# HKUST-Aerial-Robotics/VINS-Mobile

Hardware: AMD Instinct MI355X
Metric: VIO frames/sec (KLT+window solve), 640x480/150 feats/W=10 (higher is better)
Workload: dtype f64 (solve) / u8+i32+f32 (KLT)

## Files before the change

### vins-mobile_amd/csrc/marg_core.h

```cpp
#pragma once

#include "solver_core.h"

namespace vio {

struct MargOut {
  int *n;
  int *kind, *index, *offset;
  double *x0;
  double *J;
  double *r;
  double *scratch;
  int ncap;
};

template <class MP>
struct MargWorkT {
  MP Am;
  int ld;
  ldsd bm;
  ldsd tol;
  ldsd ldinv;
  ldsd hff, gf, einv;
  ldsd prdx, prr;
// ... 329 lines not shown
    }
    const int mdrop = pos;
    auto keep = [&](int kind, int idx, int col, int new_index) {
      out.kind[nblocks] = kind, out.index[nblocks] = new_index, out.offset[nblocks] = col - mdrop;
      double *x0 = out.x0 + 9 * nblocks;
      for (int q = 0; q < 9; q++) x0[q] = 0.0;
      cldsd src = kind == 0 ? xpose + 7 * idx : kind == 1 ? xsb + 9 * idx : ex;
      int gs = kind == 1 ? 9 : 7;
      for (int q = 0; q < gs; q++) x0[q] = src[q];
      nblocks++;
    };
    for (int i = 0; i < P; i++)
      if (m.col_pose[i] == -2) {
        m.col_pose[i] = pos;
        keep(0, i, pos, flag == 0 ? i - 1 : (i == W ? W - 1 : i));
        pos += 6;
      }
    for (int i = 0; i < P; i++)
      if (m.col_sb[i] == -2) {
        m.col_sb[i] = pos;
        keep(1, i, pos, flag == 0 ? i - 1 : (i == W ? W - 1 : i));
        pos += 9;
      }
    if (m.col_ex[0] == -2) {
      m.col_ex[0] = pos;
      keep(2, 0, pos, 0);
      pos += 6;
    }
    m.meta[0] = pos, m.meta[1] = mdrop, m.meta[2] = pos - mdrop, m.meta[3] = nblocks;
  }
  VIO_SYNC();
  const int pos = m.meta[0], mdrop = m.meta[1], n = m.meta[2], nblocks = m.meta[3];
  const int ld = m.ld;
  if (pos > ld || n > out.ncap) {
    if (cx.tid == 0) out.n[0] = -2, out.n[1] = 0, out.n[2] = mdrop, out.n[3] = pos;
    return;
  }
  VIO_PARFOR(q, (int)tri_doubles(pos)) m.Am[q] = 0.0;
  VIO_PARFOR(q, pos) m.bm[q] = 0.0;
  VIO_PARFOR(f, F) m.hff[f] = 0.0, m.gf[f] = 0.0;
  if (flag == 0) VIO_PARFOR(q, 12 * F) {
    const int f = q / 12, c = q - 12 * f;
    v.WTf[(size_t)f * v.n6cap + (c < 6 ? c : 6 * P + c - 6)] = 0.0;
  }
  VIO_SYNC();
  if (pn > 0) {
    VIO_PARFOR(b, v.prior_nb) {
      int kind = v.pr_kind[b], idx = v.pr_index[b], o = v.pr_offset[b];
      const double *x0 = v.pr_x0 + 9 * b;
      int base = kind == 0 ? m.col_pose[idx] : kind == 1 ? m.col_sb[idx] : m.col_ex[0];
      int ls = kind == 1 ? 9 : 6;
      for (int k = 0; k < ls; k++) m.pcol[o + k] = base + k;
      if (kind == 0) prior_block_dx(7, xpose + 7 * idx, x0, m.prdx + o);
      else if (kind == 1) prior_block_dx(9, xsb + 9 * idx, x0, m.prdx + o);
      else prior_block_dx(7, ex, x0, m.prdx + o);
    }
    VIO_PARFOR(i, pn) m.prr[i] = v.prb0[i];
    VIO_SYNC();
    dense_matvec_cols(cx, v.prH0, pn, m.prdx, [&](int i, double sacc) { VIO_ATOMIC_ADD(m.prr + i, sacc); });
    {
      constexpr int kU = 12;
      const int nst = (pn + kU - 1) / kU;
      VIO_PARFOR(q, pn * nst) {
        const int a = q / nst, b0 = kU * (q - a * nst);
        const int ca = m.pcol[a];
        double x[kU];
#pragma unroll
        for (int u = 0; u < kU; u++) x[u] = v.prH0[a * pn + (b0 + u < pn ? b0 + u : b0)];
        VIO_SCHED_FENCE();
#pragma unroll
        for (int u = 0; u < kU; u++) {
          if (b0 + u >= pn) continue;
          const int cb = m.pcol[b0 + u];
          if (ca >= cb) m.Am[tri_at(ca, cb)] = x[u];
        }
      }
    }
    VIO_SYNC();
    VIO_PARFOR(a, pn) m.bm[m.pcol[a]] += m.prr[a];
    VIO_SYNC();
  }
  stamp(cx, ST_M_PRIOR);
  if (flag == 0) {
    if (cx.tid == 0)
      imu_eval_raw(v.gravity, v.preint, xpose, xsb, xpose + 7, xsb + 9, v.imu_r, v.imu_J);
    VIO_SYNC();
    VIO_PARFOR(r, 15) {
      const double *info = v.imu_info + r * 15;
      double s = 0;
      for (int k = 0; k < 15; k++) s += info[k] * v.imu_r[k];
      v.imu_Mr[r] = s;
    }
    VIO_PARFOR(q, 450) {
      int r = q / 30, c = q % 30;
      const double *info = v.imu_info + r * 15;
      double s = 0;
      for (int k = 0; k < 15; k++) s += info[k] * v.imu_J[k * 30 + c];
      v.imu_M[q] = s;
    }
    VIO_SYNC();
    VIO_PARFOR(q, 900) {
      int a = q / 30, b = q % 30;
      int ca = a < 6 ? m.col_pose[0] + a : a < 15 ? m.col_sb[0] + a - 6 : a < 21 ? m.col_pose[1] + a - 15 : m.col_sb[1] + a - 21;
      int cb = b < 6 ? m.col_pose[0] + b : b < 15 ? m.col_sb[0] + b - 6 : b < 21 ? m.col_pose[1] + b - 15 : m.col_sb[1] + b - 21;
      double s = 0;
      for (int k = 0; k < 15; k++) s += v.imu_J[k * 30 + a] * v.imu_M[k * 30 + b];
      if (ca >= cb) VIO_ATOMIC_ADD(m.Am + tri_at(ca, cb), s);
    }
    VIO_PARFOR(a, 30) {
      int ca = a < 6 ? m.col_pose[0] + a : a < 15 ? m.col_sb[0] + a - 6 : a < 21 ? m.col_pose[1] + a - 15 : m.col_sb[1] + a - 21;
      double s = 0;
      for (int k = 0; k < 15; k++) s += v.imu_J[k * 30 + a] * v.imu_Mr[k];
      VIO_ATOMIC_ADD(m.bm + ca, s);
    }
    stamp(cx, ST_M_IMU);
    const double cc = 1.0 / v.cauchy_b;
    int S0 = 0, nb0 = 0;
    for (int p = 0; p < v.npairs && v.pair_h[p] == 0; p++)
      if (v.pair_t[p] != P) S0 = (v.pair_s1[p] + 1) & ~1, nb0 = p + 1;
    auto G = m.stage;
    const int CH = m.stage_slots;
    if (CH < 2) {
      if (cx.tid == 0) out.n[0] = -3, out.n[1] = 0;
      return;
    }
    auto add_lower = [&](int ra, int ca, double val) {
      if (ra >= ca) VIO_ATOMIC_ADD(m.Am + tri_at(ra, ca), val);
      else VIO_ATOMIC_ADD(m.Am + tri_at(ca, ra), val);
    };
    const int lane_d = VIO_TID(cx) & 63;
    const bool dv = lane_d < nb0;
    const int d_s0 = dv ? v.pair_s0[lane_d] : 0, d_s1 = dv ? v.pair_s1[lane_d] : 0;
    const int d_t = dv ? ((v.pair_h[lane_d] != 0 || v.pair_t[lane_d] == P) ? -1 : v.pair_t[lane_d]) : -1;
    for (int c0 = 0; c0 < S0; c0 += CH) {
      VIO_PARFOR(slot, (S0 - c0 < CH ? S0 - c0 : CH)) {
        const int rec = v.srec_i[c0 + slot];
        double pij[6];
#pragma unroll
        for (int c = 0; c < 6; c++) pij[c] = v.srec_d[6 * (size_t)(c0 + slot) + c];
        if (rec < 0) continue;
        const int t = (rec >> 8) & 255, f = rec >> 16;
        if ((rec & 255) != 0 || t == P) continue;
        double r[2], Ji[12], Jj[12], Jex[12], Jl[2];
        projection_eval(v.s_info, xpose, xpose + 7 * t, ex, xfeat[f], pij, pij + 3, true, r, Ji, Jj, Jex, Jl);
        double sq = r[0] * r[0] + r[1] * r[1];
        double sr = sqrt(1.0 / (1.0 + sq * cc));
        auto g = G + slot * kMargSlot; auto gx = g + kSlotStride;
#pragma unroll
        for (int rr = 0; rr < 2; rr++) {
#pragma unroll
          for (int c = 0; c < 6; c++) {
            g[rr * kRowLen + c] = Ji[rr * 6 + c] * sr, g[rr * kRowLen + 6 + c] = Jj[rr * 6 + c] * sr;
            gx[rr * kMargRowX + c] = Jex[rr * 6 + c] * sr;
          }
          g[rr * kRowLen + 12] = r[rr] * sr, g[rr * kRowLen + 13] = Jl[rr] * sr;
        }
        const double s2 = sr * sr;
        double *wf = v.WTf + (size_t)f * v.n6cap;
#pragma unroll
        for (int c = 0; c < 6; c++) {
          wf[6 * t + c] = (Jj[c] * Jl[0] + Jj[6 + c] * Jl[1]) * s2;
          VIO_ATOMIC_ADD(wf + c, (Ji[c] * Jl[0] + Ji[6 + c] * Jl[1]) * s2);
          VIO_ATOMIC_ADD(wf + 6 * P + c, (Jex[c] * Jl[0] + Jex[6 + c] * Jl[1]) * s2);
        }
        VIO_ATOMIC_ADD(m.hff + f, (Jl[0] * Jl[0] + Jl[1] * Jl[1]) * s2);
        VIO_ATOMIC_ADD(m.gf + f, (Jl[0] * r[0] + Jl[1] * r[1]) * s2);
      }
      VIO_SYNC();
// ... 127 lines not shown
```

### vins-mobile_amd/csrc/solver_core.h

```cpp
#pragma once

#include <math.h>
#include <stdint.h>

#include <type_traits>

#include "vio_math.h"

#if defined(VIO_EMUL) || defined(VIO_SIMT)
#define VIO_HOST_BUILD 1
#endif
#ifdef VIO_HOST_BUILD
#define VIO_DEV inline
#define VIO_ATOMIC_ADD(p, v) ::vio::atomic_add((p), (v))
#else
#define VIO_DEV __device__ __forceinline__
#define VIO_ATOMIC_ADD(p, v) ::vio::atomic_add((p), (v))
#endif
#if defined(VIO_EMUL)
#define VIO_SYNC() ((void)0)
#define VIO_SYNC_LDS() ((void)0)
#elif defined(VIO_SIMT)
#define VIO_SYNC() __syncthreads()
#define VIO_SYNC_LDS() __syncthreads()
// ... 552 lines not shown
  const double sum_dt = pre[0];
  const double *delta_p = pre + 1, *delta_q = pre + 4, *delta_v = pre + 8, *lin_ba = pre + 11, *lin_bg = pre + 14;
  const double *J = pre + 17;
  PA Pi = pose_i, Pj = pose_j, Vi = sb_i, Bai = sb_i + 3, Bgi = sb_i + 6, Vj = sb_j, Baj = sb_j + 3, Bgj = sb_j + 6;
  Quat Qi{pose_i[3], pose_i[4], pose_i[5], pose_i[6]}, Qj{pose_j[3], pose_j[4], pose_j[5], pose_j[6]};
  Quat dq{delta_q[0], delta_q[1], delta_q[2], delta_q[3]};
  double dp_dba[9], dp_dbg[9], dq_dbg[9], dv_dba[9], dv_dbg[9];
  for (int i = 0; i < 3; i++)
    for (int j = 0; j < 3; j++) {
      dp_dba[i * 3 + j] = J[(0 + i) * 15 + 9 + j];
      dp_dbg[i * 3 + j] = J[(0 + i) * 15 + 12 + j];
      dq_dbg[i * 3 + j] = J[(3 + i) * 15 + 12 + j];
      dv_dba[i * 3 + j] = J[(6 + i) * 15 + 9 + j];
      dv_dbg[i * 3 + j] = J[(6 + i) * 15 + 12 + j];
    }
  double dba[3], dbg[3], th[3], t1[3], t2[3], cdv[3], cdp[3];
  for (int k = 0; k < 3; k++) dba[k] = Bai[k] - lin_ba[k], dbg[k] = Bgi[k] - lin_bg[k];
  mat3vec(dq_dbg, dbg, th);
  Quat cdq = qmul(dq, Quat{th[0] / 2.0, th[1] / 2.0, th[2] / 2.0, 1.0});
  mat3vec(dv_dba, dba, t1), mat3vec(dv_dbg, dbg, t2);
  for (int k = 0; k < 3; k++) cdv[k] = delta_v[k] + t1[k] + t2[k];
  mat3vec(dp_dba, dba, t1), mat3vec(dp_dbg, dbg, t2);
  for (int k = 0; k < 3; k++) cdp[k] = delta_p[k] + t1[k] + t2[k];
  const double T = sum_dt;
  const double G[3] = {0, 0, gravity};
  Quat Qi_inv = qinv(Qi);
  double a[3], b[3], ra[3], rb[3];
  for (int k = 0; k < 3; k++) {
    a[k] = 0.5 * G[k] * T * T + Pj[k] - Pi[k] - Vi[k] * T;
    b[k] = G[k] * T + Vj[k] - Vi[k];
  }
  qrot(Qi_inv, a, ra), qrot(Qi_inv, b, rb);
  Quat qr = qmul(qinv(cdq), qmul(Qi_inv, Qj));
  for (int k = 0; k < 3; k++) {
    res[0 + k] = ra[k] - cdp[k];
    res[6 + k] = rb[k] - cdv[k];
    res[9 + k] = Baj[k] - Bai[k];
    res[12 + k] = Bgj[k] - Bgi[k];
  }
  res[3] = 2 * qr.x, res[4] = 2 * qr.y, res[5] = 2 * qr.z;
  if (!Jraw) return;
  double Rinv[9], M[9], S[9], Mq[9];
  qtoR(Qi_inv, Rinv);
  const int ld = 30, cpi = 0, csi = 6, cpj = 15, csj = 21;
  for (int i = 0; i < 3; i++)
    for (int j = 0; j < 3; j++) Jraw[(0 + i) * ld + cpi + j] = -Rinv[i * 3 + j];
  skew3(ra, S);
  for (int i = 0; i < 3; i++)
    for (int j = 0; j < 3; j++) Jraw[(0 + i) * ld + cpi + 3 + j] = S[i * 3 + j];
  qleft_qright33(qmul(qinv(Qj), Qi), cdq, M);
  for (int i = 0; i < 3; i++)
    for (int j = 0; j < 3; j++) Jraw[(3 + i) * ld + cpi + 3 + j] = -M[i * 3 + j];
  skew3(rb, S);
  for (int i = 0; i < 3; i++)
    for (int j = 0; j < 3; j++) Jraw[(6 + i) * ld + cpi + 3 + j] = S[i * 3 + j];
  for (int i = 0; i < 3; i++)
    for (int j = 0; j < 3; j++) {
      Jraw[(0 + i) * ld + csi + 0 + j] = -Rinv[i * 3 + j] * T;
      Jraw[(0 + i) * ld + csi + 3 + j] = -dp_dba[i * 3 + j];
      Jraw[(0 + i) * ld + csi + 6 + j] = -dp_dbg[i * 3 + j];
      Jraw[(6 + i) * ld + csi + 0 + j] = -Rinv[i * 3 + j];
      Jraw[(6 + i) * ld + csi + 3 + j] = -dv_dba[i * 3 + j];
      Jraw[(6 + i) * ld + csi + 6 + j] = -dv_dbg[i * 3 + j];
      Jraw[(9 + i) * ld + csi + 3 + j] = -(double)(i == j);
      Jraw[(12 + i) * ld + csi + 6 + j] = -(double)(i == j);
    }
  qleft33(qmul(qmul(qinv(Qj), Qi), cdq), M);
  mat3mul(M, dq_dbg, Mq);
  for (int i = 0; i < 3; i++)
    for (int j = 0; j < 3; j++) Jraw[(3 + i) * ld + csi + 6 + j] = -Mq[i * 3 + j];
  for (int i = 0; i < 3; i++)
    for (int j = 0; j < 3; j++) Jraw[(0 + i) * ld + cpj + j] = Rinv[i * 3 + j];
  qleft33(qmul(qmul(qinv(cdq), Qi_inv), Qj), M);
  for (int i = 0; i < 3; i++)
    for (int j = 0; j < 3; j++) Jraw[(3 + i) * ld + cpj + 3 + j] = M[i * 3 + j];
  for (int i = 0; i < 3; i++)
    for (int j = 0; j < 3; j++) {
      Jraw[(6 + i) * ld + csj + 0 + j] = Rinv[i * 3 + j];
      Jraw[(9 + i) * ld + csj + 3 + j] = (double)(i == j);
      Jraw[(12 + i) * ld + csj + 6 + j] = (double)(i == j);
    }
}

template <class PX, class PD>
VIO_DEV void prior_block_dx(int gsize, PX x, const double *x0, PD dx) {
  if (gsize != 7) {
    for (int k = 0; k < gsize; k++) dx[k] = x[k] - x0[k];
    return;
  }
  for (int k = 0; k < 3; k++) dx[k] = x[k] - x0[k];
  Quat q = qmul(qinv(qfrom_pose(x0)), Quat{x[3], x[4], x[5], x[6]});
  double sgn = (q.w >= 0) ? 1.0 : -1.0;
  dx[3] = sgn * 2.0 * q.x, dx[4] = sgn * 2.0 * q.y, dx[5] = sgn * 2.0 * q.z;
}


#ifdef VIO_EMUL
template <class MP>
VIO_DEV void setup_imu_info(const Ctx &cx, const WinView &v, MP) {
  const int W = v.W;
  VIO_PARFOR(q, W * 450) {
    int f = q / 450, e = q % 450, r = e / 30, c = e % 30;
    v.imu_aug[q] = c < 15 ? v.preint[f * kPreintDoubles + 242 + r * 15 + c] : (double)(c - 15 == r);
  }
  VIO_SYNC();
  for (int c = 0; c < 15; c++) {
    VIO_PARFOR(f, W) {
      double *A = v.imu_aug + f * 450;
      int piv = c;
      for (int r = c + 1; r < 15; r++)
        if (fabs(A[r * 30 + c]) > fabs(A[piv * 30 + c])) piv = r;
      if (piv != c)
        for (int j = 0; j < 30; j++) {
          double t = A[c * 30 + j];
          A[c * 30 + j] = A[piv * 30 + j];
          A[piv * 30 + j] = t;
        }
      double d = A[c * 30 + c];
      for (int j = 0; j < 30; j++) A[c * 30 + j] /= d;
      for (int r = 0; r < 15; r++) v.imu_Mr[f * 15 + r] = A[r * 30 + c];
    }
    VIO_SYNC();
    VIO_PARFOR(q, W * 450) {
      int f = q / 450, e = q % 450, r = e / 30, j = e % 30;
      if (r != c) {
        double fac = v.imu_Mr[f * 15 + r];
        if (fac != 0.0) v.imu_aug[q] -= fac * v.imu_aug[f * 450 + c * 30 + j];
      }
    }
    VIO_SYNC();
  }
  VIO_PARFOR(q, W * 225) {
    int f = q / 225, e = q % 225, r = e / 15, c = e % 15;
    int rr = r >= c ? r : c, cc = r >= c ? c : r;
    v.imu_info[q] = v.imu_aug[f * 450 + rr * 30 + 15 + cc];
  }
  VIO_PARFOR(q, W * 450) v.imu_J[q] = 0.0;
  VIO_SYNC();
}
#else
template <class MP>
VIO_DEV void setup_imu_info_gj(const Ctx &cx, const WinView &v, MP mbox) {
  const int W = v.W;
  const int tid_ = VIO_TID(cx), j = tid_ & 31, slot = tid_ >> 5, nslots = cx.nt >> 5;
  for (int f0 = 0; f0 < W; f0 += nslots) {
    const int f = f0 + slot;
    const bool act = f < W && j < 30;
    const int fc = f < W ? f : 0;
    auto mb = mbox + slot * 32;
    double x[15];
#pragma unroll
    for (int r = 0; r < 15; r++)
      x[r] = j < 15 ? v.preint[fc * kPreintDoubles + 242 + r * 15 + (j < 15 ? j : 0)] : (double)(j - 15 == r);
#pragma unroll
    for (int c = 0; c < 15; c++) {
      if (j == c) {
        int piv = c;
        double best = fabs(x[c]);
#pragma unroll
        for (int r = c + 1; r < 15; r++)
          if (fabs(x[r]) > best) best = fabs(x[r]), piv = r;
#pragma unroll
        for (int r = 0; r < 15; r++) mb[r] = x[r];
        mb[15] = (double)piv;
      }
      __builtin_amdgcn_fence(__ATOMIC_RELEASE, "wavefront");
// ... 393 lines not shown
    const bool ok = m < nvalid && n < nvalid;
    const int hi = m > n ? m : n, lo = m > n ? n : m;
    A[r] = D[ok ? hi * ld + lo : 0];
  }
  tile_load_op_raw(Lprev, ld, nvalid, n, kq, l);
  VIO_SCHED_FENCE();
#pragma unroll
  for (int r = 0; r < 4; r++) {
    const int m = kq + 4 * r;
    A[r] = (m < nvalid && n < nvalid) ? A[r] : 0.0;
    E[r] = (m == n) ? 1.0 : 0.0;
  }
  if (with_update) {
    tile_mask_op(nvalid, n, l);
#pragma unroll
    for (int s = 0; s < 4; s++) A = mfma_f64(-l[s], l[s], A);
  }
  double keep[4] = {0.0, 0.0, 0.0, 0.0}, myinv = 0.0;
  double dcc = lane_bcast(A[0], 0);
#pragma unroll
  for (int c = 0; c < 16; c++) {
    if (c < npiv) {
      double y = __builtin_amdgcn_rsq(dcc);
      const double h = 0.5 * dcc;
      y = y * fma(-h * y, y, 1.5);
      const bool sel = kq == (c & 3);
      const double a = sel ? A[c >> 2] * y : 0.0;
      const double e = sel ? E[c >> 2] * y : 0.0;
      keep[c >> 2] = sel ? (n >= c ? a : e) : keep[c >> 2];
      myinv = (n == c) ? y : myinv;
      if (c + 1 < 16) {
        const double lnext = lane_bcast(a, 16 * (c & 3) + c + 1);
        const double dold = lane_bcast(A[(c + 1) >> 2], 16 * ((c + 1) & 3) + c + 1);
        dcc = fma(-lnext, lnext, dold);
      }
      A = mfma_f64(-a, a, A);
      E = mfma_f64(-a, e, E);
    }
  }
  if (n < nvalid) {
#pragma unroll
    for (int j = 0; j < 4; j++) {
      const int c = kq + 4 * j;
      if (c < npiv) D[n * ld + c] = keep[j];
    }
    if (kq == 0 && n < npiv) ldinv_k[n] = myinv;
  }
  const bool bad = n < npiv && !(myinv > 0.0 && myinv < 1.7976931348623157e308);
  return __builtin_amdgcn_ballot_w64(bad) == 0;
}
template <class MP>
VIO_DEV void tile_trsm(MP Aik, int ld_i, int rows, MP Dkk, int ld_k, cldsd ldinv_k, int li, int kq) {
  double a[4], x[4];
  tile_load_op_raw(Aik, ld_i, rows, li, kq, a);
  const double dg = ldinv_k[li];
#pragma unroll
  for (int s = 0; s < 4; s++) x[s] = Dkk[(4 * s + kq) * ld_k + li];
  VIO_SCHED_FENCE();
  tile_mask_op(rows, li, a);
  v4d acc = {0.0, 0.0, 0.0, 0.0};
#pragma unroll
  for (int s = 0; s < 4; s++) {
    const int kk = 4 * s + kq;
    const double bb = kk < li ? x[s] : (kk == li ? dg : 0.0);
    acc = mfma_f64(a[s], bb, acc);
  }
  tile_store_acc(Aik, ld_i, rows, li, kq, acc);
}
template <class MP>
VIO_DEV void tile_update(MP C, int ld_i, int rows_i, MP A, MP B, int ld_j, int rows_j, int li, int kq) {
  double a[4], b[4];
  tile_load_op_raw(A, ld_i, rows_i, li, kq, a), tile_load_op_raw(B, ld_j, rows_j, li, kq, b);
  v4d acc = tile_load_acc_raw(C, ld_i, rows_i, li, kq);
  VIO_SCHED_FENCE();
  tile_mask_op(rows_i, li, a), tile_mask_op(rows_j, li, b);
  acc = tile_mask_acc(acc, rows_i, kq);
#pragma unroll
  for (int s = 0; s < 4; s++) acc = mfma_f64(-a[s], b[s], acc);
  tile_store_acc(C, ld_i, rows_i, li, kq, acc);
}
template <class MP>
VIO_DEV void setup_imu_info(const Ctx &cx, const WinView &v, MP mbox) {
  const int W = v.W;
  VIO_PARFOR(q, W * 450) v.imu_J[q] = 0.0;
  constexpr int kLd = 17, kTile = 16 * kLd + 16;
  const int tid_ = VIO_TID(cx), wave = __builtin_amdgcn_readfirstlane(tid_ >> 6), nw = cx.nt >> 6, lane = tid_ & 63;
  const int n = lane & 15, kq = lane >> 4;
  auto T = mbox + wave * kTile;
  auto ldv = T + 16 * kLd;
  bool all_good = true;
  if (cx.tid == 0) mbox[nw * kTile] = 0.0;
  VIO_SYNC();
  for (int f = wave; f < W; f += nw) {
    const double *cov = v.preint + f * kPreintDoubles + 242;
    double c4[4];
#pragma unroll
    for (int r = 0; r < 4; r++) {
      const int row = kq + 4 * r, hi = row > n ? row : n, lo = row > n ? n : row;
      c4[r] = cov[(hi < 15 ? hi : 0) * 15 + (lo < 15 ? lo : 0)];
    }
#pragma unroll
    for (int r = 0; r < 4; r++) {
      const int row = kq + 4 * r;
      T[row * kLd + n] = (row < 15 && n < 15) ? c4[r] : (row == n ? 1.0 : 0.0);
    }
    __builtin_amdgcn_fence(__ATOMIC_RELEASE, "wavefront");
    __builtin_amdgcn_wave_barrier();
    __builtin_amdgcn_fence(__ATOMIC_ACQUIRE, "wavefront");
    const bool good = potrf16_wave(T, T, kLd, 15, 15, false, ldv, lane);
    all_good = all_good && good;
    __builtin_amdgcn_fence(__ATOMIC_RELEASE, "wavefront");
    __builtin_amdgcn_wave_barrier();
    __builtin_amdgcn_fence(__ATOMIC_ACQUIRE, "wavefront");
    double x[4];
    const double dg = ldv[n < 15 ? n : 0];
#pragma unroll
    for (int s4 = 0; s4 < 4; s4++) x[s4] = T[(n < 15 ? n : 0) * kLd + (4 * s4 + kq)];
    VIO_SCHED_FENCE();
    v4d acc = {0.0, 0.0, 0.0, 0.0};
#pragma unroll
    for (int s4 = 0; s4 < 4; s4++) {
      const int k = 4 * s4 + kq;
      const double xv = (n < 15 && k < 15) ? (k > n ? x[s4] : (k == n ? dg : 0.0)) : 0.0;
      acc = mfma_f64(xv, xv, acc);
    }
#pragma unroll
    for (int r = 0; r < 4; r++) {
      const int row = kq + 4 * r;
      if (row < 15 && n < 15) v.imu_info[f * 225 + row * 15 + n] = acc[r];
    }
    __builtin_amdgcn_wave_barrier();
  }
  if (__builtin_amdgcn_ballot_w64(!all_good) != 0 && lane == 0) mbox[nw * kTile] = 1.0;
  VIO_SYNC();
  const bool fallback = mbox[nw * kTile] == 1.0;
  VIO_SYNC();
  if (fallback) setup_imu_info_gj(cx, v, mbox);
}
#endif

#ifndef VIO_EMUL
constexpr int kPanelTiles = 5;
constexpr int kRowLen = 14;
constexpr int kSlotStride = 29;
constexpr int kGRow = 10;
constexpr int kGSlot = 2 * kGRow + 1;
constexpr int kGramPiece = 30;
constexpr int kGramMinChunk = 32;

template <class WK>
VIO_DEV int gram_chunk_slots(const Ctx &cx, const WK &w) {
  int CH = (w.nstage / kGSlot) & ~1;
  if (CH >= (int)cx.nt) CH -= CH % (int)cx.nt;
  return CH;
}

template <class WK>
VIO_DEV void build_gram_pieces(const Ctx &cx, const WinView &v, WK &w) {
  const int CH = gram_chunk_slots(cx, w), nchunks = (v.nslots + CH - 1) / CH;
  ldsi cnt = reinterpret_cast<ldsi>(w.stage);
  ldsi cc = cnt + v.npairs;
  VIO_PARFOR(c, nchunks + 1) cc[c] = 0;
  VIO_SYNC();
  VIO_PARFOR(b, v.npairs) {
    const int s0 = v.pair_s0[b], s1 = v.pair_s1[b];
    int n = 0;
    for (int c = s0 / CH; c * CH < s1; c++) {
// ... 162 lines not shown
#pragma unroll
      for (int r4 = 0; r4 < 4; r4++) {
        const int row = kq + 4 * r4;
        sgn[r4] = ((row >= 6 && row < 9) != (li >= 6 && li < 9)) ? -1.0 : 1.0;
      }
      auto gl = G + (kq >> 1) * kGSlot + (kq & 1) * kGRow + src;
      auto issue = [&](int desc, double (&a)[8]) {
        const int off = desc & 1023, n = (desc >> 10) & 31, last = ((n + 1) >> 1) - 1;
        auto g = gl + off * kGSlot;
#pragma unroll
        for (int j = 0; j < 8; j++) a[j] = g[(j < last ? j : last) * 2 * kGSlot];
      };
      auto consume = [&](int desc, double (&a)[8]) {
        const int n = (desc >> 10) & 31, h = (desc >> 15) & 63, t = (desc >> 21) & 63;
        const int total = (n + 1) >> 1;
        const int full = n >> 1;
        v4d acc = {0.0, 0.0, 0.0, 0.0};
        double xo = 0.0;
        if (n & 1) xo = kq < 2 ? a[full < 8 ? 7 : 0] : 0.0;
#pragma unroll
        for (int j = 0; j < 8; j++) {
          if (j < full) acc = mfma_f64(a[j], a[j], acc);
        }
        if (kGramPiece > 16 && total > 8) {
          const int off = desc & 1023, last = total - 1;
          auto g = gl + off * kGSlot;
          double a2[8];
#pragma unroll
          for (int j = 0; j < 8; j++) a2[j] = g[(8 + j < last ? 8 + j : last) * 2 * kGSlot];
          VIO_SCHED_FENCE();
          if (n & 1) xo = kq < 2 ? a2[7] : 0.0;
#pragma unroll
          for (int j = 0; j < 8; j++) {
            if (8 + j < full) acc = mfma_f64(a2[j], a2[j], acc);
          }
        }
        if (n & 1) acc = mfma_f64(xo, xo, acc);
#pragma unroll
        for (int r4 = 0; r4 < 4; r4++) {
          const double val = acc[r4] * sgn[r4];
          if (f_lds[r4]) VIO_ATOMIC_ADD(f_base[r4] + (f_t[r4] ? t : h) * f_mul[r4], val);
          if (f_glb[r4]) {
            const int rt = 6 * t + kq + 4 * r4 - 6, ch = 6 * h + li;
            atomic_add_noret(v.PP + (t > h ? tri_at(rt, ch) : tri_at(ch, rt)), val);
          }
        }
      };
      for (int pb = p_lo + wave; pb < p_hi; pb += 64 * nw) {
        const int pl = pb + lane * nw;
        const int m_desc = pb == p_lo + wave ? m_desc0 : (pl < p_hi ? v.gpiece[pl] : 0);
        const int cnt = (p_hi - pb + nw - 1) / nw < 64 ? (p_hi - pb + nw - 1) / nw : 64;
        double A[8], Bq[8];
        issue(__builtin_amdgcn_readlane(m_desc, 0), A);
        for (int k = 0; k < cnt; k += 2) {
          const int d0 = __builtin_amdgcn_readlane(m_desc, k);
          const int d1 = k + 1 < cnt ? __builtin_amdgcn_readlane(m_desc, k + 1) : 0;
          if (k + 1 < cnt) issue(d1, Bq);
          VIO_SCHED_FENCE();
          consume(d0, A);
          if (k + 1 < cnt) {
            if (k + 2 < cnt) issue(__builtin_amdgcn_readlane(m_desc, k + 2), A);
            VIO_SCHED_FENCE();
            consume(d1, Bq);
          }
        }
      }
    }
    VIO_SYNC();
    stamp(cx, ST_P_GRAM);
    stamp(cx, ST_P_FEAT);
  }
  if (!host_tail) return cost;
  VIO_PARFOR(f, v.F) {
    const int h = w.fh[f];
    if (h >= 0)
      for (int c = 0; c < 6; c++) {
        const double val = whv[c][f];
        v.WTf[(size_t)f * v.n6cap + 6 * h + c] = val;
      }
  }
  return cost;
}

template <class WK>
VIO_DEV double evaluate(const Ctx &cx, const WinView &v, WK &w, cldsd pose, cldsd sb,
                        cldsd feat, bool jac, bool have_scale = false, bool reuse_aux = false, bool keep_aux = false) {
  const int np = v.np;
  double cost = 0.0;
  VIO_PARFOR(i, v.P + v.has_loop + 1) {
    const bool is_ex = i == v.P + v.has_loop;
    double R[9];
    if (is_ex) qtoR(Quat{w.ex[3], w.ex[4], w.ex[5], w.ex[6]}, R);
    else qtoR(Quat{pose[7 * i + 3], pose[7 * i + 4], pose[7 * i + 5], pose[7 * i + 6]}, R);
    auto dst = w.rot + 9 * (is_ex ? v.P + 1 : i);
    for (int k = 0; k < 9; k++) dst[k] = R[k];
  }
  if (jac) {
    const int nF = v.P + v.has_loop;
    VIO_PARFOR(q, np) w.gp[q] = 0.0;
    VIO_PARFOR(q, v.F) {
      w.gf[q] = 0.0, w.hff[q] = 0.0;
      w.cfeat[q] = w.stf[q] = w.gnf[q] = w.tf[q] = w.ef[q] = w.einv[q] = 0.0;
    }
    if (!have_scale) {
      VIO_PARFOR(q, v.F * v.n6cap) v.WTf[q] = 0.0;
    }
    VIO_PARFOR(q, nF * 36) w.ppd[q] = 0.0;
    VIO_SYNC();
#ifndef VIO_HOST_BUILD
    if (cx.coop > 1) {
      const CoopLayout L = CoopLayout::make(v.Pcap, v.Fcap, v.nblk_cap);
      const int nFr = v.P + v.has_loop;
      VIO_PARFOR(q, 7 * nFr) v.coop[L.o_pose + q] = pose[q];
      VIO_PARFOR(q, v.F) v.coop[L.o_feat + q] = feat[q];
      VIO_PARFOR(q, 7) v.coop[L.o_ex + q] = w.ex[q];
      coop_post(cx, v, COOP_EVAL);
      cost += projections_jac(cx, v, w, pose, feat, have_scale, 0, cx.coop, false);
      coop_wait_helpers(cx, v);
      ldsd whv[6] = {w.cfeat, w.stf, w.gnf, w.tf, w.ef, w.einv};
      const size_t fs = ((size_t)v.Fcap + 7) & ~(size_t)7;
      for (int m = 1; m < cx.coop; m++) {
        const double *pr = v.coop + L.o_part + (size_t)(m - 1) * L.part;
        VIO_PARFOR(q, np) w.gp[q] += pr[L.p_gp + q];
        VIO_PARFOR(q, nFr * 36) w.ppd[q] += pr[L.p_ppd + q];
        VIO_PARFOR(f, v.F) {
          w.hff[f] += pr[L.p_f + f], w.gf[f] += pr[L.p_f + fs + f];
#pragma unroll
          for (int c = 0; c < 6; c++) whv[c][f] += pr[L.p_f + (2 + c) * fs + f];
        }
        if (cx.tid == 0) cost += pr[L.p_cost];
      }
      VIO_SYNC();
      VIO_PARFOR(f, v.F) {
        const int h = w.fh[f];
        if (h >= 0)
          for (int c = 0; c < 6; c++) v.WTf[(size_t)f * v.n6cap + 6 * h + c] = whv[c][f];
      }
    } else
#endif
    {
      stamp(cx, ST_E_HEAD);
      cost += projections_jac(cx, v, w, pose, feat, have_scale);
    }
    stamp(cx, ST_EVAL_PROJ);
    const int napp = (int)tri_doubles(v.nrows), nband = 2 * v.P * kSS;
    const int n = v.prior_n, nt_ = (int)cx.nt;
    const bool do_prior = n > 0 && !reuse_aux;
    {
      const int tid_ = VIO_TID(cx);
      {
        constexpr int kU = 12;
        const bool pr = n > 0;
        for (int q0 = tid_; q0 < napp; q0 += kU * nt_) {
          double x[kU], y[kU];
#pragma unroll
          for (int u = 0; u < kU; u++) {
            const int q = q0 + u * nt_, qc = q < napp ? q : 0;
            x[u] = pr ? v.AppPr[qc] : 0.0, y[u] = v.PP[qc];
          }
          VIO_SCHED_FENCE();
#pragma unroll
          for (int u = 0; u < kU; u++) {
            const int q = q0 + u * nt_;
            if (q < napp) w.App[q] = x[u] + y[u], v.PP[q] = 0.0;
          }
        }
        for (int q0 = tid_; q0 < nband; q0 += kU * nt_) {
          double x[kU];
#pragma unroll
          for (int u = 0; u < kU; u++) {
            const int q = q0 + u * nt_;
            x[u] = pr ? v.AppPr[napp + (q < nband ? q : 0)] : 0.0;
          }
          VIO_SCHED_FENCE();
#pragma unroll
          for (int u = 0; u < kU; u++) {
            const int q = q0 + u * nt_;
            if (q < nband) w.Dss[q] = x[u];
          }
        }
      }
      VIO_PARFOR(q, v.P * kAS) w.AspI[q] = 0.0;
      if (w.asp_ring) {
        if (tid_ < 4) w.aspring[2 * kAS + tid_] = 0.0;
      } else if (w.asp_lds && tid_ < 16) {
        w.AspI[v.Pcap * kAS + tid_] = 0.0;
      }
      if (do_prior) {
        VIO_PARFOR(b, v.prior_nb) {
          int kind = v.pr_kind[b], idx = v.pr_index[b], o = v.pr_offset[b];
          const double *x0 = v.pr_x0 + 9 * b;
          if (kind == 0) prior_block_dx(7, pose + 7 * idx, x0, w.prdx + o);
          else if (kind == 1) prior_block_dx(9, sb + 9 * idx, x0, w.prdx + o);
          else prior_block_dx(7, w.ex, x0, w.prdx + o);
        }
        VIO_PARFOR(i, n) w.prr[i] = v.prb0[i];
      }
      if (!reuse_aux) {
        const int f = nt_ - 1 - tid_;
        if (f < v.W)
          imu_eval_raw(v.gravity, v.preint + f * kPreintDoubles, pose + 7 * f, sb + 9 * f, pose + 7 * (f + 1), sb + 9 * (f + 1),
                       v.imu_r + f * 15, v.imu_J + f * 450);
      }
    }
    VIO_SYNC();
    stamp(cx, ST_IMU_RAW);
    {
      const int tid_ = VIO_TID(cx);
      constexpr int kStrip = 25;
      int nparts = do_prior ? nt_ / n : 1;
      const int need = (n + 4 * kStrip - 1) / (4 * kStrip);
      nparts = nparts < need ? need : (nparts > 8 ? 8 : nparts);
      const int per = do_prior ? (n + nparts - 1) / nparts : 0;
      const bool one_strip = do_prior && n * nparts <= nt_ && per <= kStrip;
      if (one_strip && tid_ < n * nparts) {
        const int hpart = tid_ / n, hc = tid_ - hpart * n;
        const int hk0 = hpart * per, hnb = hk0 + per < n ? per : n - hk0;
        if (hnb > 0) {
          double hs[kStrip], sacc = 0;
#pragma unroll
          for (int j = 0; j < kStrip; j++) hs[j] = v.prH0[(size_t)(hk0 + (j < hnb ? j : 0)) * n + hc];
          VIO_SCHED_FENCE();
#pragma unroll
          for (int j = 0; j < kStrip; j++) sacc += (j < hnb ? hs[j] : 0.0) * w.prdx[hk0 + (j < hnb ? j : 0)];
          VIO_ATOMIC_ADD(w.prr + hc, sacc);
        }
      }
      if (do_prior && !one_strip)
        dense_matvec_cols(cx, v.prH0, n, w.prdx, [&](int i, double sacc) { VIO_ATOMIC_ADD(w.prr + i, sacc); });
      const int nF = v.P + v.has_loop;
      VIO_PARFOR(q, nF * 36) {
        const int a = q / 36, e = q - a * 36, r = e / 6, c = e - r * 6;
        if (r >= c) VIO_ATOMIC_ADD(w.App + tri_at(6 * a + r, 6 * a + c), w.ppd[q]);
      }
    }
    VIO_SYNC();
    stamp(cx, ST_EVAL_PRIOR);
    if (n > 0) VIO_PARFOR(i, n) {
      const double r0 = v.pr_r[i], b0 = v.prb0[i];
      cost += 0.5 * r0 * r0 + 0.5 * w.prdx[i] * (w.prr[i] + b0);
      const int pa = w.prcol[i];
      if (pa >= 0) VIO_ATOMIC_ADD(w.gp + kBS * (pa >> 8) + (pa & 255), w.prr[i]);
    }
    {
      const int tid_ = VIO_TID(cx), wave = tid_ >> 6, nw = cx.nt >> 6, lane = tid_ & 63;
      const int n = lane & 15, kq = lane >> 4;
      struct ImuOps {
        double a[4], b0[4], b1[4];
      };
      auto imu_fetch = [&](int f, ImuOps &o) {
        const double *info = v.imu_info + f * 225, *Jr = v.imu_J + f * 450, *rr = v.imu_r + f * 15;
#pragma unroll
        for (int s4 = 0; s4 < 4; s4++) {
          const int k = 4 * s4 + kq, kc = k < 15 ? k : 0;
          o.a[s4] = info[(n < 15 ? n : 0) * 15 + kc];
          o.b0[s4] = Jr[kc * 30 + n];
          o.b1[s4] = n == 14 ? rr[kc] : Jr[kc * 30 + 16 + (n < 14 ? n : 0)];
        }
      };
      ImuOps nxt;
      if (wave < v.W) imu_fetch(wave, nxt);
      for (int f = wave; f < v.W; f += nw) {
        const ImuOps cur = nxt;
        if (f + nw < v.W) imu_fetch(f + nw, nxt);
        VIO_SCHED_FENCE();
        double av[4], bv[2][4];
#pragma unroll
        for (int s4 = 0; s4 < 4; s4++) {
          const bool kok = 4 * s4 + kq < 15;
          av[s4] = (kok && n < 15) ? cur.a[s4] : 0.0;
          bv[0][s4] = kok ? cur.b0[s4] : 0.0;
          bv[1][s4] = (kok && n < 15) ? cur.b1[s4] : 0.0;
        }
        v4d T0 = {0, 0, 0, 0}, T1 = {0, 0, 0, 0};
#pragma unroll
        for (int s4 = 0; s4 < 4; s4++) T0 = mfma_f64(av[s4], bv[0][s4], T0), T1 = mfma_f64(av[s4], bv[1][s4], T1);
        v4d G00 = {0, 0, 0, 0}, G10 = {0, 0, 0, 0}, G11 = {0, 0, 0, 0};
#pragma unroll
        for (int s4 = 0; s4 < 4; s4++) {
          G00 = mfma_f64(bv[0][s4], T0[s4], G00);
          G10 = mfma_f64(bv[1][s4], T0[s4], G10);
          G11 = mfma_f64(bv[1][s4], T1[s4], G11);
        }
#pragma unroll
        for (int r4 = 0; r4 < 4; r4++) {
          const int row = kq + 4 * r4;
          if (row >= n) red_put(v, w, f + (row >= 15), row >= 15 ? row - 15 : row, f + (n >= 15), n >= 15 ? n - 15 : n, G00[r4], true);
          const int R = 16 + row;
          if (R < 30) {
            red_put(v, w, f + 1, R - 15, f + (n >= 15), n >= 15 ? n - 15 : n, G10[r4], true);
            if (n < 14 && R >= 16 + n) red_put(v, w, f + 1, R - 15, f + 1, n + 1, G11[r4], true);
          } else if (R == 30) {
            VIO_ATOMIC_ADD(w.gp + 15 * f + n, G10[r4]);
            if (n < 14) VIO_ATOMIC_ADD(w.gp + 15 * f + 16 + n, G11[r4]);
            if (n == 14) cost += 0.5 * G11[r4];
          }
        }
      }
    }
    VIO_SYNC();
    stamp(cx, ST_EVAL_IMU);
  } else {
    const int n = v.prior_n;
    if (n > 0 && !reuse_aux) {
      VIO_PARFOR(b, v.prior_nb) {
        int kind = v.pr_kind[b], idx = v.pr_index[b], o = v.pr_offset[b];
        const double *x0 = v.pr_x0 + 9 * b;
        if (kind == 0) prior_block_dx(7, pose + 7 * idx, x0, w.prdx + o);
        else if (kind == 1) prior_block_dx(9, sb + 9 * idx, x0, w.prdx + o);
        else prior_block_dx(7, w.ex, x0, w.prdx + o);
      }
      VIO_PARFOR(i, n) w.prr[i] = v.prb0[i];
      VIO_SYNC();
      dense_matvec_cols(cx, v.prH0, n, w.prdx, [&](int i, double sacc) { VIO_ATOMIC_ADD(w.prr + i, sacc); });
    }
    VIO_SYNC();
    if (n > 0) VIO_PARFOR(i, n) {
      const double r0 = v.pr_r[i], b0 = v.prb0[i];
      cost += 0.5 * r0 * r0 + 0.5 * w.prdx[i] * (w.prr[i] + b0);
    }
    stamp(cx, ST_COST_EVAL);
    if (!reuse_aux) {
      VIO_PARFOR(f, v.W) {
        imu_eval_raw(v.gravity, v.preint + f * kPreintDoubles, pose + 7 * f, sb + 9 * f, pose + 7 * (f + 1),
                     sb + 9 * (f + 1), v.imu_r + f * 15, keep_aux ? v.imu_J + f * 450 : nullptr);
      }
      VIO_SYNC();
    }
    stamp(cx, ST_D0);
    VIO_PARFOR(q, v.W * 15) {
      int f = q / 15, r = q % 15;
      const double *info = v.imu_info + f * 225 + r * 15;
      const double *rr = v.imu_r + f * 15;
      double s = 0;
      for (int k = 0; k < 15; k++) s += info[k] * rr[k];
      cost += 0.5 * s * rr[r];
    }
    stamp(cx, ST_D1);
    const double bb = v.cauchy_b, cc = 1.0 / bb;
    int sl = VIO_TID(cx);
    int rec = sl < v.nslots ? v.srec_i[sl] : -1;
    double pij[6];
#pragma unroll
    for (int c = 0; c < 6; c++) pij[c] = v.srec_d[6 * (size_t)(sl < v.nslots ? sl : 0) + c];
    while (sl < v.nslots) {
      const int nx = sl + (int)cx.nt;
      const int rec_n = nx < v.nslots ? v.srec_i[nx] : -1;
      double pn[6];
#pragma unroll
      for (int c = 0; c < 6; c++) pn[c] = v.srec_d[6 * (size_t)(nx < v.nslots ? nx : 0) + c];
      if (rec >= 0) {
        const int h = rec & 255, t = (rec >> 8) & 255, f = rec >> 16;
        double r[2];
        projection_eval_rot(v.s_info, w.rot + 9 * h, pose + 7 * h, w.rot + 9 * t, pose + 7 * t, w.rot + 9 * (v.P + 1), w.ex,
                            feat[f], pij, pij + 3, false, r, nullptr, nullptr, nullptr);
        cost += 0.5 * bb * log(1.0 + (r[0] * r[0] + r[1] * r[1]) * cc);
      }
      sl = nx, rec = rec_n;
#pragma unroll
      for (int c = 0; c < 6; c++) pij[c] = pn[c];
    }
    stamp(cx, ST_D2);
  }
  double total = block_sum(cx, cost);
  if (jac) {
    VIO_PARFOR(i, np) {
      const int f = i / kBS, c = i - f * kBS;
      const double h = c < 6 ? w.App[tri_at(6 * f + c, 6 * f + c)] : w.Dss[f * kSS + (c - 6) * (kSB + 1)];
      if (!have_scale) w.sp[i] = rcp_f(1.0 + sqrt_f(h));
      const double sc = w.sp[i];
      w.dp[i] = sqrt_f(fmin(fmax(sc * sc * h, 1e-6), 1e32));
    }
    VIO_SYNC();
  }
  stamp(cx, ST_COST_EVAL);
  return total;
}


template <class WK>
VIO_DEV double feat_d2(const WK &w, int f) {
  return fmin(fmax(w.sf[f] * w.sf[f] * w.hff[f], 1e-6), 1e32);
}
template <class WK>
VIO_DEV double feat_d(const WK &w, int f) {
  return sqrt_f(feat_d2(w, f));
}
template <class WK>
VIO_DEV double feat_gd(const WK &w, int f) {
  return w.sf[f] * w.gf[f] * rsqrt_f(feat_d2(w, f));
}

template <class WK>
VIO_DEV double pose_gd(const WK &w, int i) {
  return w.sp[i] * w.gp[i] * rcp_f(w.dp[i]);
}

template <class WK>
VIO_DEV double quad_form_H(const Ctx &cx, const WinView &v, WK &w, cldsd vp, cldsd vf, bool prepared = false, bool w_part = true) {
  const int np = v.np, F = v.F, n6 = v.n6, P = v.P;
  if (!prepared) {
    VIO_PARFOR(f, F) w.tf[f] = 0.0;
    VIO_PARFOR(i, np) {
      const int f = i / kBS, c = i - f * kBS;
      const double u = w.sp[i] * vp[i];
      w.t1[i] = u;
      if (c < 6) w.xt[6 * f + c] = u;
    }
    VIO_SYNC();
// ... 1724 lines not shown
```

Baseline: 185,700.

## Evaluate IMU residuals and Jacobians across quad lanes with DPP shuffles

Replaces the one-thread-per-frame IMU residual/Jacobian evaluation with a lane-parallel version where each group of four lanes handles one frame. Quaternion components are exchanged via DPP quad moves. Constant Jacobian entries are now written once during info setup instead of on every evaluation. The goal is to shorten the serial per-thread IMU evaluation on the critical path, including the single-thread marginalization call, at the cost of more complex code and reliance on the constant entries having been written beforehand.

```diff
diff --git a/vins-mobile_amd/csrc/marg_core.h b/vins-mobile_amd/csrc/marg_core.h
--- a/vins-mobile_amd/csrc/marg_core.h
+++ b/vins-mobile_amd/csrc/marg_core.h
@@ -435,8 +435,15 @@
   }
   stamp(cx, ST_M_PRIOR);
   if (flag == 0) {
+#ifdef VIO_EMUL
     if (cx.tid == 0)
       imu_eval_raw(v.gravity, v.preint, xpose, xsb, xpose + 7, xsb + 9, v.imu_r, v.imu_J);
+#else
+    {
+      const int tid_ = VIO_TID(cx);
+      if (tid_ < 64) imu_eval_lanes(tid_, tid_ < 4, v.gravity, v.preint, xpose, xsb, xpose + 7, xsb + 9, v.imu_r, v.imu_J, true);
+    }
+#endif
     VIO_SYNC();
     VIO_PARFOR(r, 15) {
       const double *info = v.imu_info + r * 15;
diff --git a/vins-mobile_amd/csrc/solver_core.h b/vins-mobile_amd/csrc/solver_core.h
--- a/vins-mobile_amd/csrc/solver_core.h
+++ b/vins-mobile_amd/csrc/solver_core.h
@@ -658,6 +658,174 @@
     }
 }
 
+VIO_DEV double imu_J_const(const double *pre, int r, int c) {
+  if (c >= 9 && c < 15 && (r < 3 || (r >= 6 && r < 9))) return -pre[17 + r * 15 + c];
+  if (r >= 9) {
+    const int b = r >= 12 ? 12 : 9;
+    if (c >= b && c < b + 3) return -(double)(c == r);
+    if (c >= b + 15 && c < b + 18) return (double)(c == r + 15);
+  }
+  return 0.0;
+}
+
+#ifndef VIO_EMUL
+constexpr int kQpB0 = 0x00, kQpB1 = 0x55, kQpB2 = 0xAA, kQpB3 = 0xFF;
+constexpr int kQpR1 = 0xC9, kQpR2 = 0xD2;
+template <int CTRL>
+VIO_DEV double quad_get(double v) {
+  return dpp_move_f64<CTRL, 0xf>(v);
+}
+struct LaneQ {
+  double s, r1, r2, w;
+};
+struct LaneV {
+  double s, r1, r2;
+};
+VIO_DEV LaneQ laneq(double s) { return LaneQ{s, quad_get<kQpR1>(s), quad_get<kQpR2>(s), quad_get<kQpB3>(s)}; }
+VIO_DEV LaneV lanev(double s) { return LaneV{s, quad_get<kQpR1>(s), quad_get<kQpR2>(s)}; }
+VIO_DEV double laneq_mul(const LaneQ &a, const LaneQ &b, bool c3) {
+  const double xyz = a.w * b.s + a.s * b.w + a.r1 * b.r2 - a.r2 * b.r1;
+  const double p = a.s * b.s;
+  const double p0 = quad_get<kQpB0>(p), p1 = quad_get<kQpB1>(p), p2 = quad_get<kQpB2>(p);
+  const double ww = a.w * b.w - p0 - p1 - p2;
+  return c3 ? ww : xyz;
+}
+VIO_DEV LaneQ laneq_inv(const LaneQ &q, bool c3) {
+  const double sq = q.s * q.s;
+  const double n2 = quad_get<kQpB0>(sq) + quad_get<kQpB1>(sq) + quad_get<kQpB2>(sq) + quad_get<kQpB3>(sq);
+  const double s = c3 ? q.s : -q.s, r1 = c3 ? q.r1 : -q.r1, r2 = c3 ? q.r2 : -q.r2;
+#ifdef VIO_FAST_F64
+  const double in = rcp_f(n2);
+  return LaneQ{s * in, r1 * in, r2 * in, q.w * in};
+#else
+  return LaneQ{s / n2, r1 / n2, r2 / n2, q.w / n2};
+#endif
+}
+VIO_DEV double laneq_rot(const LaneQ &q, const LaneV &v) {
+  const double u = 2 * (q.r1 * v.r2 - q.r2 * v.r1);
+  const double u1 = 2 * (q.r2 * v.s - q.s * v.r2), u2 = 2 * (q.s * v.r1 - q.r1 * v.s);
+  return v.s + q.w * u + (q.r1 * u2 - q.r2 * u1);
+}
+VIO_DEV void cyc_to_nat(int c, double k0, double k1, double k2, double n[3]) {
+  n[0] = c == 1 ? k2 : (c == 2 ? k1 : k0);
+  n[1] = c == 1 ? k0 : (c == 2 ? k2 : k1);
+  n[2] = c == 1 ? k1 : (c == 2 ? k0 : k2);
+}
+
+template <class PA>
+VIO_DEV void imu_eval_lanes(int lane, bool act, double gravity, const double *pre, PA pose_i, PA sb_i, PA pose_j, PA sb_j,
+                            double *res, double *Jraw, bool write_const) {
+  const int c = lane & 3;
+  const bool c3 = c == 3;
+  const int cc = c3 ? 2 : c;
+  const bool st = act && !c3;
+  const double *J = pre + 17;
+  const double T = pre[0], delta_p = pre[1 + cc], delta_q = pre[4 + c], delta_v = pre[8 + cc], lin_ba = pre[11 + cc],
+               lin_bg = pre[14 + cc];
+  double dp_dba[3], dp_dbg[3], dq_dbg_r[3], dv_dba[3], dv_dbg[3], Dq[9];
+#pragma unroll
+  for (int j = 0; j < 3; j++) {
+    dp_dba[j] = J[(0 + cc) * 15 + 9 + j], dp_dbg[j] = J[(0 + cc) * 15 + 12 + j], dq_dbg_r[j] = J[(3 + cc) * 15 + 12 + j];
+    dv_dba[j] = J[(6 + cc) * 15 + 9 + j], dv_dbg[j] = J[(6 + cc) * 15 + 12 + j];
+  }
+  if (Jraw) {
+#pragma unroll
+    for (int i = 0; i < 3; i++)
+#pragma unroll
+      for (int j = 0; j < 3; j++) Dq[i * 3 + j] = J[(3 + i) * 15 + 12 + j];
+  }
+  const double Pi = pose_i[cc], Pj = pose_j[cc], Vi = sb_i[cc], Bai = sb_i[3 + cc], Bgi = sb_i[6 + cc], Vj = sb_j[cc],
+               Baj = sb_j[3 + cc], Bgj = sb_j[6 + cc];
+  const LaneQ Qi = laneq(pose_i[3 + c]), Qj = laneq(pose_j[3 + c]), dq = laneq(delta_q);
+  const double dba = Bai - lin_ba, dbg = Bgi - lin_bg;
+  const double a0 = quad_get<kQpB0>(dba), a1 = quad_get<kQpB1>(dba), a2 = quad_get<kQpB2>(dba);
+  const double g0 = quad_get<kQpB0>(dbg), g1 = quad_get<kQpB1>(dbg), g2 = quad_get<kQpB2>(dbg);
+  const double th = dq_dbg_r[0] * g0 + dq_dbg_r[1] * g1 + dq_dbg_r[2] * g2;
+  const LaneQ cdq = laneq(laneq_mul(dq, laneq(c3 ? 1.0 : th / 2.0), c3));
+  double t1 = dv_dba[0] * a0 + dv_dba[1] * a1 + dv_dba[2] * a2, t2 = dv_dbg[0] * g0 + dv_dbg[1] * g1 + dv_dbg[2] * g2;
+  const double cdv = delta_v + t1 + t2;
+  t1 = dp_dba[0] * a0 + dp_dba[1] * a1 + dp_dba[2] * a2, t2 = dp_dbg[0] * g0 + dp_dbg[1] * g1 + dp_dbg[2] * g2;
+  const double cdp = delta_p + t1 + t2;
+  const double Gc = c == 2 ? gravity : 0.0;
+  const LaneQ Qi_inv = laneq_inv(Qi, c3);
+  const LaneV a = lanev(0.5 * Gc * T * T + Pj - Pi - Vi * T), b = lanev(Gc * T + Vj - Vi);
+  const double ra = laneq_rot(Qi_inv, a), rb = laneq_rot(Qi_inv, b);
+  const LaneQ cdq_inv = laneq_inv(cdq, c3);
+  const double qr = laneq_mul(cdq_inv, laneq(laneq_mul(Qi_inv, Qj, c3)), c3);
+  if (st) {
+    res[0 + c] = ra - cdp, res[3 + c] = 2 * qr, res[6 + c] = rb - cdv;
+    res[9 + c] = Baj - Bai, res[12 + c] = Bgj - Bgi;
+  }
+  if (!Jraw) return;
+  const int ld = 30, cpi = 0, csi = 6, cpj = 15, csj = 21;
+  const int k1 = c >= 2 ? c - 2 : c + 1, k2 = c >= 1 ? c - 1 : c + 2;
+  const int col[3] = {cc, c3 ? 0 : k1, c3 ? 1 : k2};
+  {
+    const LaneQ &q = Qi_inv;
+    const double tr1 = 2 * q.r1, tr2 = 2 * q.r2;
+    const double R[3] = {1 - (tr1 * q.r1 + tr2 * q.r2), tr1 * q.s - tr2 * q.w, tr2 * q.s + tr1 * q.w};
+    if (st) {
+#pragma unroll
+      for (int k = 0; k < 3; k++) {
+        Jraw[(0 + c) * ld + cpi + col[k]] = -R[k];
+        Jraw[(0 + c) * ld + csi + col[k]] = -R[k] * T;
+        Jraw[(6 + c) * ld + csi + col[k]] = -R[k];
+        Jraw[(0 + c) * ld + cpj + col[k]] = R[k];
+        Jraw[(6 + c) * ld + csj + col[k]] = R[k];
+      }
+    }
+  }
+  {
+    const LaneV va = lanev(ra), vb = lanev(rb);
+    if (st) {
+      Jraw[(0 + c) * ld + cpi + 3 + col[1]] = -va.r2, Jraw[(0 + c) * ld + cpi + 3 + col[2]] = va.r1;
+      Jraw[(6 + c) * ld + cpi + 3 + col[1]] = -vb.r2, Jraw[(6 + c) * ld + cpi + 3 + col[2]] = vb.r1;
+      if (write_const) Jraw[(0 + c) * ld + cpi + 3 + col[0]] = 0.0, Jraw[(6 + c) * ld + cpi + 3 + col[0]] = 0.0;
+    }
+  }
+  const LaneQ QjiQi = laneq(laneq_mul(laneq_inv(Qj, c3), Qi, c3));
+  {
+    double L[3];
+    cyc_to_nat(cc, QjiQi.w, -QjiQi.r2, QjiQi.r1, L);
+    const double b0 = quad_get<kQpB0>(cdq.s), b1 = quad_get<kQpB1>(cdq.s), b2 = quad_get<kQpB2>(cdq.s), bw = cdq.w;
+    const double Rm[9] = {bw, b2, -b1, -b2, bw, b0, b1, -b0, bw};
+    const double nb[3] = {-b0, -b1, -b2};
+#pragma unroll
+    for (int j = 0; j < 3; j++) {
+      double m = L[0] * Rm[j] + L[1] * Rm[3 + j] + L[2] * Rm[6 + j];
+      m += QjiQi.s * nb[j];
+      if (st) Jraw[(3 + c) * ld + cpi + 3 + j] = -m;
+    }
+  }
+  {
+    const LaneQ q = laneq(laneq_mul(QjiQi, cdq, c3));
+    double M[3];
+    cyc_to_nat(cc, q.w, -q.r2, q.r1, M);
+#pragma unroll
+    for (int j = 0; j < 3; j++) {
+      const double m = M[0] * Dq[j] + M[1] * Dq[3 + j] + M[2] * Dq[6 + j];
+      if (st) Jraw[(3 + c) * ld + csi + 6 + j] = -m;
+    }
+  }
+  {
+    const LaneQ q = laneq(laneq_mul(laneq(laneq_mul(cdq_inv, Qi_inv, c3)), Qj, c3));
+    if (st) {
+      Jraw[(3 + c) * ld + cpj + 3 + col[0]] = q.w;
+      Jraw[(3 + c) * ld + cpj + 3 + col[1]] = -q.r2;
+      Jraw[(3 + c) * ld + cpj + 3 + col[2]] = q.r1;
+    }
+  }
+  if (st && write_const) {
+#pragma unroll
+    for (int j = 0; j < 3; j++) {
+      Jraw[(0 + c) * ld + csi + 3 + j] = -dp_dba[j], Jraw[(0 + c) * ld + csi + 6 + j] = -dp_dbg[j];
+      Jraw[(6 + c) * ld + csi + 3 + j] = -dv_dba[j], Jraw[(6 + c) * ld + csi + 6 + j] = -dv_dbg[j];
+      Jraw[(9 + c) * ld + csi + 3 + j] = -(double)(c == j), Jraw[(12 + c) * ld + csi + 6 + j] = -(double)(c == j);
+      Jraw[(9 + c) * ld + csj + 3 + j] = (double)(c == j), Jraw[(12 + c) * ld + csj + 6 + j] = (double)(c == j);
+    }
+  }
+}
+#endif
 template <class PX, class PD>
 VIO_DEV void prior_block_dx(int gsize, PX x, const double *x0, PD dx) {
   if (gsize != 7) {
@@ -1217,7 +1385,10 @@
 template <class MP>
 VIO_DEV void setup_imu_info(const Ctx &cx, const WinView &v, MP mbox) {
   const int W = v.W;
-  VIO_PARFOR(q, W * 450) v.imu_J[q] = 0.0;
+  VIO_PARFOR(q, W * 450) {
+    const int f = q / 450, e = q - 450 * f, r = e / 30;
+    v.imu_J[q] = imu_J_const(v.preint + f * kPreintDoubles, r, e - 30 * r);
+  }
   constexpr int kLd = 17, kTile = 16 * kLd + 16;
   const int tid_ = VIO_TID(cx), wave = __builtin_amdgcn_readfirstlane(tid_ >> 6), nw = cx.nt >> 6, lane = tid_ & 63;
   const int n = lane & 15, kq = lane >> 4;
@@ -1546,6 +1717,26 @@
   return cost;
 }
 
+template <class PA>
+VIO_DEV void imu_raw_all(const Ctx &cx, const WinView &v, PA pose, PA sb, bool want_J) {
+#ifdef VIO_EMUL
+  VIO_PARFOR(f, v.W)
+    imu_eval_raw(v.gravity, v.preint + f * kPreintDoubles, pose + 7 * f, sb + 9 * f, pose + 7 * (f + 1), sb + 9 * (f + 1),
+                 v.imu_r + f * 15, want_J ? v.imu_J + f * 450 : nullptr);
+#else
+  const int tid_ = VIO_TID(cx), lane = tid_ & 63, nw = (int)cx.nt >> 6, wave = __builtin_amdgcn_readfirstlane(tid_ >> 6);
+  const int npass = (v.W + 15) >> 4;
+  for (int p = 0; p < npass; p++) {
+    if (nw - 1 - p % nw != wave) continue;
+    const int fq = 16 * p + (lane >> 2);
+    const bool act = fq < v.W;
+    const int f = act ? fq : v.W - 1;
+    imu_eval_lanes(lane, act, v.gravity, v.preint + f * kPreintDoubles, pose + 7 * f, sb + 9 * f, pose + 7 * (f + 1),
+                   sb + 9 * (f + 1), v.imu_r + f * 15, want_J ? v.imu_J + f * 450 : nullptr, false);
+  }
+#endif
+}
+
 template <class WK>
 VIO_DEV double evaluate(const Ctx &cx, const WinView &v, WK &w, cldsd pose, cldsd sb,
                         cldsd feat, bool jac, bool have_scale = false, bool reuse_aux = false, bool keep_aux = false) {
@@ -1660,12 +1851,7 @@
         }
         VIO_PARFOR(i, n) w.prr[i] = v.prb0[i];
       }
-      if (!reuse_aux) {
-        const int f = nt_ - 1 - tid_;
-        if (f < v.W)
-          imu_eval_raw(v.gravity, v.preint + f * kPreintDoubles, pose + 7 * f, sb + 9 * f, pose + 7 * (f + 1), sb + 9 * (f + 1),
-                       v.imu_r + f * 15, v.imu_J + f * 450);
-      }
+      if (!reuse_aux) imu_raw_all(cx, v, pose, sb, true);
     }
     VIO_SYNC();
     stamp(cx, ST_IMU_RAW);
@@ -1785,10 +1971,7 @@
     }
     stamp(cx, ST_COST_EVAL);
     if (!reuse_aux) {
-      VIO_PARFOR(f, v.W) {
-        imu_eval_raw(v.gravity, v.preint + f * kPreintDoubles, pose + 7 * f, sb + 9 * f, pose + 7 * (f + 1),
-                     sb + 9 * (f + 1), v.imu_r + f * 15, keep_aux ? v.imu_J + f * 450 : nullptr);
-      }
+      imu_raw_all(cx, v, pose, sb, keep_aux);
       VIO_SYNC();
     }
     stamp(cx, ST_D0);
```

After: 187,200 (median of 6 runs). About the same (+0.8%).
